# allenai/satlas-super-resolution

Hardware: AMD Instinct MI355X
Metric: G+D train-step images/sec (higher is better)
Workload: dtype fp32h

## Files before the change

### satlas_super_resolution_amd/csrc/conv_big_x3.hip

```cpp
#include "common.h"
#include <cstdlib>

namespace {

constexpr int XB_TH = 32, XB_TW = 16;
template <int KT> struct XbT {
    static constexpr int AROW = 80;
    static constexpr int VPP = 4;
    static constexpr int PH = XB_TH + KT - 1, PW = XB_TW + KT - 1, NPIX = PH * PW;
    static constexpr int PATCH = NPIX * AROW;
    static constexpr int WROWS = KT * KT * 64;
    static constexpr int WBYTES = WROWS * AROW;
    static constexpr int BUF = PATCH + WBYTES;
    static constexpr int BIAS = BUF;
    static constexpr int SLABS = BIAS + 256;
    static constexpr int LDS = SLABS + 4 * 32 * 272;
    static constexpr int NPV = (NPIX * VPP + 255) / 256;
    static constexpr int NWV = (WROWS * VPP + 255) / 256;
    static constexpr int NSTEP = KT * KT;
    static constexpr int TAIL = KT == 3 ? 2 : 1;
    static constexpr int LPS = (NPV + NWV + NSTEP - TAIL - 1) / (NSTEP - TAIL);
    static_assert(LDS <= 160 * 1024 && LPS <= 6, "LDS budget / load slots of a step");
};

#define XB_BAR() asm volatile("s_waitcnt lgkmcnt(0)\n\ts_barrier" ::: "memory")
#ifdef SSR_PROBE
#define XB_T() (__builtin_amdgcn_s_memtime())
#define XB_ACC(k, t0) do { const unsigned long long t1_ = XB_T(); xb_t[k] += t1_ - (t0); (t0) = t1_; } while (0)
#else
#define XB_T() 0ull
#define XB_ACC(k, t0) do { } while (0)
#endif
constexpr int XB_OOB = 0x7ffffff0;
constexpr int XB_SLAB_PITCH = 272, XB_SLAB = 32 * XB_SLAB_PITCH;
__device__ __forceinline__ __amdgpu_buffer_rsrc_t xb_rsrc(const void* p, long bytes) {
    return __builtin_amdgcn_make_buffer_rsrc(const_cast<void*>(p), 0, (int)(bytes > 0x7fffff00L ? 0x7fffff00L : (bytes < 0 ? 0 : bytes)), 0x00020000);
}
template <int KT>
__device__ __forceinline__ void xb_pixel(int w, int m, int s, int& row, int& col) {
    row = 8 * w + 2 * m + (s >> 4);
    col = s < 16 ? s : ((s + 32 - (XB_TW + KT - 1)) & 15);
}
__device__ __forceinline__ void xb_split4(const u32x4& v, uint2& hi, uint2& lo) {
    const f32x4 f = __builtin_bit_cast(f32x4, v);
    bf16x4 h, l;
#pragma unroll
    for (int k = 0; k < 4; ++k) {
        h[k] = (__bf16)f[k];
        l[k] = (__bf16)(f[k] - (float)h[k]);
    }
    hi = __builtin_bit_cast(uint2, h);
    lo = __builtin_bit_cast(uint2, l);
}

template <int KT, bool H = false>
__device__ __forceinline__ void conv_bigx3_body(const ssr_conv_desc& d) {
    using T = XbT<KT>;
    constexpr int AROW = T::AROW, VPP = T::VPP, PW = T::PW, NPIX = T::NPIX, PATCH = T::PATCH, NPV = T::NPV, NWV = T::NWV, NSTEP = T::NSTEP;
    extern __shared__ __attribute__((aligned(16))) char smem[];
    const int tid = threadIdx.x, lane = tid & 63, wave = tid >> 6;
    const int i = lane & 31, g = lane >> 5;
    const int tiles_x = (d.Gw + XB_TW - 1) / XB_TW, tiles_y = (d.Gh + XB_TH - 1) / XB_TH;
    const int tpi = tiles_x * tiles_y, G = gridDim.x / tpi;
    const int tp = blockIdx.x % tpi, n0 = blockIdx.x / tpi;
    const int tx_i = tp % tiles_x, ty_i = tp / tiles_x;
    const int nimg = (d.N - n0 + G - 1) / G;
    const int gy0 = ty_i * XB_TH, gx0 = tx_i * XB_TW;
    const int co0 = blockIdx.y * 64;
    const int upshift = d.up == 2 ? 1 : 0;
    const int LH = d.Hi << upshift, LW = d.Wi << upshift;
    const int nchunks = (d.Cin + 15) / 16;
    const int wchunk = KT * KT * d.CoutPad * 64;
    const int T_ = nimg * nchunks;
    const int ximg = d.Hi * d.Wi * d.x.cs * 4, oimg = d.Ho * d.Wo;

    unsigned long long xb_t[8] = {0, 0, 0, 0, 0, 0, 0, 0}, xb_t0 = XB_T();
    const unsigned long long xb_start = xb_t0;
    (void)xb_t; (void)xb_start;
    float* bias_lds = reinterpret_cast<float*>(smem + T::BIAS);
    if (tid < 64) bias_lds[tid] = (d.bias && co0 + tid < d.Cout) ? d.bias[co0 + tid] * (H ? SSR_F32H_WSCALE : 1.f) : 0.f;

    const bool s2d = KT == 2 && d.s2d != 0;
    const int cpc_shift = s2d ? 31 - __builtin_clz((unsigned)(d.Cin >> 6)) : 0;
    const int x_cs = d.x.cs, x_Wi = d.Wi, x_Cin = d.Cin;
    static_assert((T::WROWS * VPP) % 256 == 0, "no partial weight vector");
    const int p4 = tid >> 2, part4 = tid & 3;
    const int plo0 = p4 * AROW + part4 * 8;
    const int wlo0 = PATCH + p4 * AROW + part4 * 16;
    const int wgo0 = (co0 + p4) * 64 + part4 * 16, wstep = d.CoutPad * 64;
    constexpr int PTAIL = NPIX * VPP - (NPV - 1) * 256;
    int pgo[NPV];
    unsigned pmk[KT == 2 ? NPV : 1];
    const int climit = s2d ? 0x7fffffff : x_Cin - (tid % VPP) * 4;
#pragma unroll
    for (int q = 0; q < NPV; ++q) {
        const int v = tid + q * 256;
        const int pix = v / VPP, part = v % VPP;
        const int py = pix / PW, px = pix - py * PW;
        const int ly = gy0 + py - d.pad_y, lx = gx0 + px - d.pad_x;
        if constexpr (KT == 2) {
            if (s2d) {
                const int sy = 2 * ly - 1, sx = 2 * lx - 1;
                const bool y0 = sy >= 0 && sy < d.Hi, y1 = sy + 1 >= 0 && sy + 1 < d.Hi;
                const bool x0 = sx >= 0 && sx < d.Wi, x1 = sx + 1 >= 0 && sx + 1 < d.Wi;
                pmk[q] = v < NPIX * VPP ? (unsigned)(y0 && x0) | (unsigned)(y0 && x1) << 1 | (unsigned)(y1 && x0) << 2 | (unsigned)(y1 && x1) << 3 : 0u;
                pgo[q] = ((sy * d.Wi + sx) * d.x.cs + d.x.coff + part * 4) * 4 + (d.Wi + 1) * d.x.cs * 4;
            } else {
                const bool ok = v < NPIX * VPP && ly >= 0 && ly < LH && lx >= 0 && lx < LW;
                pmk[q] = ok ? 1u : 0u;
                pgo[q] = ok ? (((ly >> upshift) * d.Wi + (lx >> upshift)) * d.x.cs + d.x.coff + part * 4) * 4 : XB_OOB;
            }
        } else {
            const bool ok = v < NPIX * VPP && ly >= 0 && ly < LH && lx >= 0 && lx < LW;
            pgo[q] = ok ? (((ly >> upshift) * d.Wi + (lx >> upshift)) * d.x.cs + d.x.coff + part * 4) * 4 : XB_OOB;
        }
    }
    const long xbias = s2d ? (long)(d.Wi + 1) * d.x.cs * 4 : 0;
    const __amdgpu_buffer_rsrc_t rsx = xb_rsrc(reinterpret_cast<const char*>(d.x.p) - xbias, (long)d.N * ximg + xbias),
                                 rsw = xb_rsrc(d.w, (long)nchunks * wchunk);
    u32x4 rp[NPV], rw[NWV];
    struct LoadPos { int q, c0, xs, ws; };
    auto load_pos = [&](int nn, int c) {
        LoadPos p;
        p.c0 = c * 16;
        if constexpr (KT == 2) {
            p.q = s2d ? c >> cpc_shift : 0;
            p.xs = nn * ximg + (s2d ? (((p.q >> 1) * x_Wi + (p.q & 1)) * x_cs + ((c - (p.q << cpc_shift)) << 4)) * 4 : p.c0 * 4);
        } else {
            p.q = 0;
            p.xs = nn * ximg + p.c0 * 4;
        }
        p.ws = c * wchunk;
        return p;
    };
    auto load_one = [&](const LoadPos& lp, auto jc) {
        constexpr int j = decltype(jc)::value;
        if constexpr (j < NPV) {
            bool ok = lp.c0 < climit;
            if constexpr (KT == 2) ok = ok && ((pmk[j] >> lp.q) & 1u);
            rp[j] = __builtin_amdgcn_raw_buffer_load_b128(rsx, ok ? pgo[j] : XB_OOB, lp.xs, 0);
        } else {
            rw[j - NPV] = __builtin_amdgcn_raw_buffer_load_b128(rsw, wgo0, lp.ws + (j - NPV) * wstep, 0);
        }
    };
    auto load_chunk = [&](int nn, int c) { const LoadPos lp = load_pos(nn, c); static_for<0, NPV + NWV>([&](auto jc) { load_one(lp, jc); }); };
    auto store_chunk = [&]() {
        static_for<0, NPV>([&](auto jc) {
            constexpr int j = decltype(jc)::value;
            uint2 hi, lo;
            split_f32x4<H>(rp[j], hi, lo);
            if (j + 1 < NPV || tid < PTAIL) {
                *reinterpret_cast<uint2*>(smem + plo0 + j * 64 * AROW) = hi;
                *reinterpret_cast<uint2*>(smem + plo0 + j * 64 * AROW + 32) = lo;
            }
        });
        static_for<0, NWV>([&](auto jc) {
            constexpr int j = decltype(jc)::value;
            *reinterpret_cast<u32x4*>(smem + wlo0 + j * 64 * AROW) = rw[j];
        });
    };

    int a_off[4];
#pragma unroll
    for (int m = 0; m < 4; ++m) {
        int row, col;
        xb_pixel<KT>(wave, m, i, row, col);
        a_off[m] = (row * PW + col) * AROW + g * 16;
    }
    const int b_off = PATCH + i * AROW + g * 16;
    const int co_l = 4 * g;

    load_chunk(n0, 0);
    __syncthreads();
    XB_ACC(1, xb_t0);
    f32x16 acc[4][2];
    auto acc_init = [&]() {
#pragma unroll
        for (int t = 0; t < 2; ++t)
#pragma unroll
            for (int q4 = 0; q4 < 4; ++q4) {
                const f32x4 bq = *reinterpret_cast<const f32x4*>(bias_lds + t * 32 + 8 * q4 + co_l);
#pragma unroll
                for (int e = 0; e < 4; ++e)
#pragma unroll
                    for (int m = 0; m < 4; ++m) acc[m][t][4 * q4 + e] = bq[e];
            }
    };

    char* slab = smem + T::SLABS + wave * XB_SLAB;
    auto epilogue_impl = [&](int nn, auto opsc, auto y01c) __attribute__((always_inline)) {
        constexpr bool OPS = decltype(opsc)::value, Y01 = decltype(y01c)::value;
        const long obytes = (long)d.N * oimg * 4;
        const __amdgpu_buffer_rsrc_t rs_r1 = xb_rsrc(d.r1.p, d.r1.p ? obytes * d.r1.cs : 0), rs_r2 = xb_rsrc(d.r2.p, d.r2.p ? obytes * d.r2.cs : 0),
                                     rs_m = xb_rsrc(d.m.p, d.m.p ? obytes * d.m.cs : 0), rs_y = xb_rsrc(d.y.p, obytes * d.y.cs),
                                     rs_y0 = xb_rsrc(d.y0.p, d.y0.p ? obytes * d.y0.cs : 0), rs_y1 = xb_rsrc(d.y1.p, d.y1.p ? obytes * d.y1.cs : 0);
        const bool has_r1 = d.r1.p != nullptr, has_r2 = d.r2.p != nullptr, has_m = d.m.p != nullptr, has_acc = d.accumulate != 0,
                   has_y0 = d.y0.p != nullptr, has_y1 = d.y1.p != nullptr, m_relu = d.m_relu != 0;
        const float slope = d.act == SSR_ACT_LRELU ? 0.2f : d.act == SSR_ACT_RELU ? 0.f : 1.f;
        const float alpha = d.alpha, beta1 = has_r1 ? d.beta1 : 0.f, beta2 = has_r2 ? d.beta2 : 0.f, gacc = has_acc ? 1.f : 0.f;
        const int y_cs = d.y.cs, y_co = d.y.coff, y0_cs = d.y0.cs, y0_co = d.y0.coff, y1_cs = d.y1.cs, y1_co = d.y1.coff;
        const int r1_cs = d.r1.cs, r1_co = d.r1.coff, r2_cs = d.r2.cs, r2_co = d.r2.coff, m_cs = d.m.cs, m_co = d.m.coff;
        const int Gh = d.Gh, Gw = d.Gw, oys = d.oys, oyo = d.oyo, oxs = d.oxs, oxo = d.oxo, Wo = d.Wo;
        const int pimg = nn * oimg;
        const int hp = lane >> 4, c = co0 + (lane & 15) * 4;
        const bool cok = c < d.Cout;
#pragma unroll
        for (int m = 0; m < 4; ++m) {
            int po[8];
#pragma unroll
            for (int h = 0; h < 8; ++h) {
                int row, col;
                xb_pixel<KT>(wave, m, 4 * h + hp, row, col);
                const int gy = gy0 + row, gx = gx0 + col;
                const bool ok = gy < Gh && gx < Gw;
                const int cy = gy < Gh ? gy : Gh - 1, cx = gx < Gw ? gx : Gw - 1;
                po[h] = (pimg + (cy * oys + oyo) * Wo + cx * oxs + oxo) | (ok && cok ? 0 : (int)0x80000000);
            }
#pragma unroll
            for (int t = 0; t < 2; ++t)
#pragma unroll
                for (int q4 = 0; q4 < 4; ++q4) {
                    const f32x4 v = {acc[m][t][4 * q4], acc[m][t][4 * q4 + 1], acc[m][t][4 * q4 + 2], acc[m][t][4 * q4 + 3]};
                    *reinterpret_cast<f32x4*>(slab + i * XB_SLAB_PITCH + (t * 32 + 8 * q4 + co_l) * 4) = v;
                }
#pragma unroll
            for (int hh = 0; hh < 2; ++hh) {
                u32x4 q1[OPS ? 4 : 1], q2[OPS ? 4 : 1], qa[OPS ? 4 : 1], qm[OPS ? 4 : 1];
                if constexpr (OPS) {
#pragma unroll
                    for (int h4 = 0; h4 < 4; ++h4) {
                        const int pp = po[4 * hh + h4] & 0x7fffffff;
                        q1[h4] = __builtin_amdgcn_raw_buffer_load_b128(rs_r1, cok && has_r1 ? (pp * r1_cs + r1_co + c) * 4 : XB_OOB, 0, 0);
                        q2[h4] = __builtin_amdgcn_raw_buffer_load_b128(rs_r2, cok && has_r2 ? (pp * r2_cs + r2_co + c) * 4 : XB_OOB, 0, 0);
                        qa[h4] = __builtin_amdgcn_raw_buffer_load_b128(rs_y, cok && has_acc ? (pp * y_cs + y_co + c) * 4 : XB_OOB, 0, 0);
                        qm[h4] = __builtin_amdgcn_raw_buffer_load_b128(rs_m, cok && has_m ? (pp * m_cs + m_co + c) * 4 : XB_OOB, 0, 0);
                    }
                }
#pragma unroll
                for (int h4 = 0; h4 < 4; ++h4) {
                    const int h = 4 * hh + h4;
                    f32x4 a = *reinterpret_cast<const f32x4*>(slab + (4 * h + hp) * XB_SLAB_PITCH + (lane & 15) * 16);
                    if constexpr (H) a *= SSR_F32H_UNSCALE;
                    const bool ok = po[h] >= 0;
                    const int pp = po[h] & 0x7fffffff;
                    f32x4 v, s0, s1;
#pragma unroll
                    for (int e = 0; e < 4; ++e) {
                        float x = fmaxf(a[e], slope * a[e]) * alpha;
                        s0[e] = x;
                        if constexpr (OPS) {
                            x += beta1 * __builtin_bit_cast(f32x4, q1[h4])[e] + beta2 * __builtin_bit_cast(f32x4, q2[h4])[e] + gacc * __builtin_bit_cast(f32x4, qa[h4])[e];
                            s1[e] = x;
                            const float mv = __builtin_bit_cast(f32x4, qm[h4])[e];
                            const float f = m_relu ? (mv > 0.f ? 1.f : 0.f) : lrelu_grad_from_out(mv);
                            x *= has_m ? f : 1.f;
                        } else {
                            s1[e] = x;
                        }
                        v[e] = x;
                    }
                    if constexpr (Y01) {
                        __builtin_amdgcn_raw_buffer_store_b128(__builtin_bit_cast(u32x4, s0), rs_y0, ok && has_y0 ? (pp * y0_cs + y0_co + c) * 4 : XB_OOB, 0, 0);
                        __builtin_amdgcn_raw_buffer_store_b128(__builtin_bit_cast(u32x4, s1), rs_y1, ok && has_y1 ? (pp * y1_cs + y1_co + c) * 4 : XB_OOB, 0, 0);
                    }
                    __builtin_amdgcn_raw_buffer_store_b128(__builtin_bit_cast(u32x4, v), rs_y, ok ? (pp * y_cs + y_co + c) * 4 : XB_OOB, 0, 0);
                }
            }
        }
    };
    auto epilogue = [&](int nn) __attribute__((always_inline)) {
        const bool ops = d.r1.p != nullptr || d.r2.p != nullptr || d.m.p != nullptr || d.accumulate != 0;
        const bool y01 = d.y0.p != nullptr || d.y1.p != nullptr;
        if (ops) {
            if (y01) epilogue_impl(nn, std::true_type{}, std::true_type{});
            else epilogue_impl(nn, std::true_type{}, std::false_type{});
        } else {
            if (y01) epilogue_impl(nn, std::false_type{}, std::true_type{});
            else epilogue_impl(nn, std::false_type{}, std::false_type{});
        }
    };

    auto chunk = [&](int c, bool stored, int nn1, int c1, auto hnc) __attribute__((always_inline)) {
        constexpr bool has_next = decltype(hnc)::value;
        xb_t0 = XB_T();
        if (!stored) {
            if (c > 0) XB_BAR();
            XB_ACC(2, xb_t0);
            store_chunk();
            XB_ACC(3, xb_t0);
        }
        XB_BAR();
        XB_ACC(4, xb_t0);
        const LoadPos lp1 = load_pos(nn1, c1);
        bf16x8 wq[2][2][2], pq[2][4][2];
        auto issue1 = [&](auto sc, auto kc) {
            constexpr int s_ = decltype(sc)::value, k = decltype(kc)::value;
            if constexpr (k < 4)
                wq[s_ & 1][k >> 1][k & 1] = *reinterpret_cast<const bf16x8*>(smem + b_off + (s_ * 64 + (k >> 1) * 32) * AROW + (k & 1) * 32);
            else
                pq[s_ & 1][(k - 4) >> 1][k & 1] =
                    *reinterpret_cast<const bf16x8*>(smem + a_off[(k - 4) >> 1] + ((s_ / KT) * PW + s_ % KT) * AROW + (k & 1) * 32);
        };
        static_for<0, 12>([&](auto kc) { issue1(std::integral_constant<int, 0>{}, kc); });
        static_for<0, NSTEP>([&](auto sc) {
            constexpr int s_ = decltype(sc)::value;
            static_for<0, 24>([&](auto kc) {
                constexpr int k = decltype(kc)::value, m = k / 6, t = (k % 6) / 3, p = k % 3;
                acc[m][t] = split_mfma<H>(wq[s_ & 1][t][p == 0 ? 1 : 0], pq[s_ & 1][m][p == 1 ? 1 : 0], acc[m][t]);
                __builtin_amdgcn_sched_barrier(0);
                if constexpr (k < 12) {
                    if constexpr (s_ + 1 < NSTEP) issue1(std::integral_constant<int, s_ + 1>{}, kc);
                } else if constexpr (has_next && (k & 1) == 0 && (k - 12) / 2 < T::LPS) {
                    constexpr int j = s_ * T::LPS + (k - 12) / 2;
                    if constexpr (j < NPV + NWV) load_one(lp1, std::integral_constant<int, j>{});
                }
                __builtin_amdgcn_sched_barrier(0);
            });
        });
        __builtin_amdgcn_sched_barrier(0);
        XB_ACC(5, xb_t0);
        xb_t[7] += 1;
    };
    int gc = 0;
    for (int k = 0; k < nimg; ++k) {
        const int nn = n0 + k * G;
        const bool last_img = k + 1 == nimg;
        acc_init();
        for (int c = 0; c < (last_img ? nchunks - 1 : nchunks); ++c, ++gc) {
            const bool last_c = c + 1 == nchunks;
            chunk(gc, k > 0 && c == 0, last_c ? nn + G : nn, last_c ? 0 : c + 1, std::true_type{});
        }
        if (!last_img) {
            xb_t0 = XB_T();
            XB_BAR();
            XB_ACC(2, xb_t0);
            store_chunk();
            XB_ACC(3, xb_t0);
            epilogue(nn);
            XB_ACC(6, xb_t0);
        }
    }
    const int nl = n0 + (nimg - 1) * G;
    chunk(gc, nimg > 1 && nchunks == 1, nl, 0, std::false_type{});
    xb_t0 = XB_T();
    epilogue(nl);
    XB_ACC(6, xb_t0);
#ifdef SSR_PROBE
    if (tid == 0) {
        xb_t[0] = XB_T() - xb_start;
        const int b = (blockIdx.z * gridDim.y + blockIdx.y) * gridDim.x + blockIdx.x;
        for (int k = 0; k < 8; ++k) g_probe[b * 8 + k] = xb_t[k];
    }
#endif
    (void)T_;
}

struct ssr_conv_desc4x { ssr_conv_desc d[4]; };
template <int KT>
__global__ __launch_bounds__(256, 1) void conv_bigx3_kernel4(const ssr_conv_desc4x p) {
    conv_bigx3_body<KT>(p.d[blockIdx.z]);
}
template <int KT>
__global__ __launch_bounds__(256, 1) void conv_bigh3_kernel4(const ssr_conv_desc4x p) {
    conv_bigx3_body<KT, true>(p.d[blockIdx.z]);
}

template <int KT, bool H = false>
int launch_bigx3(const ssr_conv_desc* ds, int n, hipStream_t st) {
    constexpr int lds = XbT<KT>::LDS;
    const ssr_conv_desc& d = ds[0];
    const int tpi = ((d.Gh + XB_TH - 1) / XB_TH) * ((d.Gw + XB_TW - 1) / XB_TW);
    static const int ncu = [] { int dev = 0, v = 256; if (hipGetDevice(&dev) == hipSuccess && hipDeviceGetAttribute(&v, hipDeviceAttributeMultiprocessorCount, dev) != hipSuccess) v = 256; return v > 0 ? v : 256; }();
    int G = d.N;
    {
        const long per_img = (long)tpi * (d.CoutPad / 64) * n;
        long best = -1;
        for (int g = 1; g <= d.N; ++g) {
            const long rounds = (per_img * g + ncu - 1) / ncu, cost = rounds * ((d.N + g - 1) / g);
            const long key = (cost << 24) | (rounds << 12) | (4095 - (g > 4095 ? 4095 : g));
            if (best < 0 || key < best) { best = key; G = g; }
        }
    }
    if (const char* e = getenv("SSR_CONV_BIG_G")) {
        const int g = atoi(e);
        if (g >= 1) G = g < d.N ? g : d.N;
    }
    const int tiles = tpi * G;
    auto kern = H ? conv_bigh3_kernel4<KT> : conv_bigx3_kernel4<KT>;
    static bool attr_done[SSR_MAX_DEVICES] = {};
    const int attr_dev = ssr_device_ordinal();
    if (!attr_done[attr_dev]) {
        hipError_t e = hipFuncSetAttribute(reinterpret_cast<const void*>(kern), hipFuncAttributeMaxDynamicSharedMemorySize, lds);
        if (e != hipSuccess) return (int)e;
        attr_done[attr_dev] = true;
    }
    ssr_conv_desc4x p;
    for (int k = 0; k < 4; ++k) p.d[k] = ds[k < n ? k : 0];
    hipLaunchKernelGGL(kern, dim3(tiles, d.CoutPad / 64, n), dim3(256), lds, st, p);
    SSR_LAUNCH_CHECK();
    return SSR_OK;
}

}

bool ssr_conv_bigx3_shape_ok(const ssr_conv_desc& d) {
    if ((d.dtype != SSR_F32X3 && d.dtype != SSR_F32H) || d.fix_list) return false;
    const bool k3 = d.KH == 3 && d.KW == 3 && d.pad_y == 1 && d.pad_x == 1;
    const bool k2 = d.KH == 2 && d.KW == 2 && (d.pad_y == 0 || d.pad_y == 1) && (d.pad_x == 0 || d.pad_x == 1);
    if (!(k3 || k2) || d.stride != 1 || d.x2.p) return false;
    if (d.Cin < 8 || (d.CoutPad % 64) != 0 || (d.Cout % 4) != 0) return false;
    if (d.s2d) {
        const int cpc = d.Cin / 64;
        if (!k2 || d.pad_y != 0 || d.pad_x != 0 || d.up != 1 || (d.Cin % 64) != 0 || cpc < 1 || (cpc & (cpc - 1)) != 0) return false;
        if ((d.Hi % 2) != 0 || (d.Wi % 2) != 0 || d.Gh != d.Hi / 2 || d.Gw != d.Wi / 2) return false;
    } else if (d.Gh != (d.Hi << (d.up == 2)) || d.Gw != (d.Wi << (d.up == 2))) return false;
    if (d.r1.p && d.r1_nc < d.Cout) return false;
    if (d.r2.p && d.r2_nc < d.Cout) return false;
    if (d.m.p && !(d.m_c0 == 0 && d.m_c1 >= d.Cout)) return false;
    const long lim = 0x7fffff00L;
    const long xin = ((long)d.N * d.Hi * d.Wi + d.Wi + 1) * d.x.cs * 4, npo = (long)d.N * d.Ho * d.Wo * 4;
    if (xin > lim || npo * d.y.cs > lim || (d.y0.p && npo * d.y0.cs > lim) || (d.y1.p && npo * d.y1.cs > lim) || (d.r1.p && npo * d.r1.cs > lim) ||
        (d.r2.p && npo * d.r2.cs > lim) || (d.m.p && npo * d.m.cs > lim))
        return false;
    if ((long)((d.Cin + 15) / 16) * d.KH * d.KW * d.CoutPad * 64 > lim) return false;
    auto al16 = [](const ssr_view& v) { return !v.p || ((v.cs % 4) == 0 && (v.coff % 4) == 0 && ((uintptr_t)v.p % 16) == 0); };
    return d.x.p && d.y.p && al16(d.x) && al16(d.y) && al16(d.y0) && al16(d.y1) && al16(d.r1) && al16(d.r2) && al16(d.m);
}

bool ssr_conv_bigx3_qualifies(const ssr_conv_desc& d) {
    static const bool off = [] { const char* e = getenv("SSR_X3_BIGTILE"); return e && e[0] == '0'; }();
    if (off || !ssr_conv_bigx3_shape_ok(d) || d.KH != 3) return false;
    const long per_img = (long)((d.Gh + XB_TH - 1) / XB_TH) * ((d.Gw + XB_TW - 1) / XB_TW) * (d.CoutPad / 64);
    return per_img >= 4 && d.Gh >= 24;
}

bool ssr_conv_bigx3_try(const ssr_conv_desc& d, hipStream_t st, int* rc, bool force) {
    if (force ? !ssr_conv_bigx3_shape_ok(d) : !ssr_conv_bigx3_qualifies(d)) return false;
    if (d.dtype == SSR_F32H) *rc = d.KH == 3 ? launch_bigx3<3, true>(&d, 1, st) : launch_bigx3<2, true>(&d, 1, st);
    else *rc = d.KH == 3 ? launch_bigx3<3>(&d, 1, st) : launch_bigx3<2>(&d, 1, st);
    return true;
}

bool ssr_conv_bigx3_batch_try(const ssr_conv_desc* ds, int n, hipStream_t st, int* rc) {
    const char* e = getenv("SSR_X3_BIGTILE2");
    const bool off = e && e[0] == '0', always = e && e[0] == '2';
    if (off || n < 1 || n > 4) return false;
    for (int k = 0; k < n; ++k)
        if (!ssr_conv_bigx3_shape_ok(ds[k]) || ds[k].dtype != SSR_F32X3 || ds[k].KH != 2 || ds[k].s2d) return false;
    const ssr_conv_desc& d = ds[0];
    for (int k = 1; k < n; ++k)
        if (ds[k].N != d.N || ds[k].Gh != d.Gh || ds[k].Gw != d.Gw || ds[k].CoutPad != d.CoutPad || ds[k].Cin != d.Cin || ds[k].Hi != d.Hi || ds[k].Wi != d.Wi ||
            ds[k].up != d.up)
            return false;
    const long per_img = (long)((d.Gh + XB_TH - 1) / XB_TH) * ((d.Gw + XB_TW - 1) / XB_TW) * (d.CoutPad / 64) * n;
    if (!always && (per_img < 8 || d.Gh < 24)) return false;
    *rc = launch_bigx3<2>(ds, n, st);
    return true;
}
```

Measured before the change: 1186.

## Double-buffer input patches in big conv kernel to overlap loads with MFMA

Adds a pipelined variant of the big conv kernel in which the input patch, and for 2x2 kernels also the weights, live in two LDS buffers. The next chunk's global loads, hi/lo split and LDS stores are interleaved with the current chunk's MFMAs, which removes the per-chunk serialisation of load, barrier and compute. The epilogue slab reuses the idle patch buffer, and the leaky-ReLU product is precomputed in one epilogue case. This is on by default through an env toggle. In exchange it raises LDS use and register pressure and adds complex scheduling.

```diff
diff --git a/satlas_super_resolution_amd/csrc/conv_big_x3.hip b/satlas_super_resolution_amd/csrc/conv_big_x3.hip
--- a/satlas_super_resolution_amd/csrc/conv_big_x3.hip
+++ b/satlas_super_resolution_amd/csrc/conv_big_x3.hip
@@ -21,6 +21,13 @@
     static constexpr int TAIL = KT == 3 ? 2 : 1;
     static constexpr int LPS = (NPV + NWV + NSTEP - TAIL - 1) / (NSTEP - TAIL);
     static_assert(LDS <= 160 * 1024 && LPS <= 6, "LDS budget / load slots of a step");
+    static constexpr bool WDB = KT == 2;
+    static constexpr int PWB = 2 * PATCH;
+    static constexpr int PBIAS = PWB + (WDB ? 2 : 1) * WBYTES;
+    static constexpr int PLDS = PBIAS + 256;
+    static constexpr int PSTEPS = (NPV + 2) / 3;
+    static_assert(PLDS <= 160 * 1024 && 4 * 32 * 272 <= PATCH && (PATCH % 16) == 0, "pipelined LDS budget / slabs in a patch buffer");
+    static_assert(PSTEPS < NSTEP && 2 * NWV <= 24, "pipelined store slots");
 };
 
 #define XB_BAR() asm volatile("s_waitcnt lgkmcnt(0)\n\ts_barrier" ::: "memory")
@@ -41,6 +48,27 @@
     row = 8 * w + 2 * m + (s >> 4);
     col = s < 16 ? s : ((s + 32 - (XB_TW + KT - 1)) & 15);
 }
+template <bool H> __device__ __forceinline__ void xb_split2(float a, float b, uint32_t& hi, uint32_t& lo) {
+    if constexpr (H) {
+        typedef _Float16 f16x2 __attribute__((ext_vector_type(2)));
+        f16x2 h, l;
+        h[0] = (_Float16)a;
+        h[1] = (_Float16)b;
+        l[0] = (_Float16)(a - (float)h[0]);
+        l[1] = (_Float16)(b - (float)h[1]);
+        hi = __builtin_bit_cast(uint32_t, h);
+        lo = __builtin_bit_cast(uint32_t, l);
+    } else {
+        typedef __bf16 bf16x2 __attribute__((ext_vector_type(2)));
+        bf16x2 h, l;
+        h[0] = (__bf16)a;
+        h[1] = (__bf16)b;
+        l[0] = (__bf16)(a - (float)h[0]);
+        l[1] = (__bf16)(b - (float)h[1]);
+        hi = __builtin_bit_cast(uint32_t, h);
+        lo = __builtin_bit_cast(uint32_t, l);
+    }
+}
 __device__ __forceinline__ void xb_split4(const u32x4& v, uint2& hi, uint2& lo) {
     const f32x4 f = __builtin_bit_cast(f32x4, v);
     bf16x4 h, l;
@@ -53,7 +81,7 @@
     lo = __builtin_bit_cast(uint2, l);
 }
 
-template <int KT, bool H = false>
+template <int KT, bool H = false, bool PIPE = false>
 __device__ __forceinline__ void conv_bigx3_body(const ssr_conv_desc& d) {
     using T = XbT<KT>;
     constexpr int AROW = T::AROW, VPP = T::VPP, PW = T::PW, NPIX = T::NPIX, PATCH = T::PATCH, NPV = T::NPV, NWV = T::NWV, NSTEP = T::NSTEP;
@@ -77,7 +105,7 @@
     unsigned long long xb_t[8] = {0, 0, 0, 0, 0, 0, 0, 0}, xb_t0 = XB_T();
     const unsigned long long xb_start = xb_t0;
     (void)xb_t; (void)xb_start;
-    float* bias_lds = reinterpret_cast<float*>(smem + T::BIAS);
+    float* bias_lds = reinterpret_cast<float*>(smem + (PIPE ? T::PBIAS : T::BIAS));
     if (tid < 64) bias_lds[tid] = (d.bias && co0 + tid < d.Cout) ? d.bias[co0 + tid] * (H ? SSR_F32H_WSCALE : 1.f) : 0.f;
 
     const bool s2d = KT == 2 && d.s2d != 0;
@@ -170,9 +198,11 @@
     const int b_off = PATCH + i * AROW + g * 16;
     const int co_l = 4 * g;
 
-    load_chunk(n0, 0);
-    __syncthreads();
-    XB_ACC(1, xb_t0);
+    if constexpr (!PIPE) {
+        load_chunk(n0, 0);
+        __syncthreads();
+        XB_ACC(1, xb_t0);
+    }
     f32x16 acc[4][2];
     auto acc_init = [&]() {
 #pragma unroll
@@ -243,10 +273,15 @@
                     if constexpr (H) a *= SSR_F32H_UNSCALE;
                     const bool ok = po[h] >= 0;
                     const int pp = po[h] & 0x7fffffff;
-                    f32x4 v, s0, s1;
+                    f32x4 v, s0, s1, s0p;
+                    if constexpr (OPS && Y01) {
+#pragma unroll
+                        for (int e = 0; e < 4; ++e) s0p[e] = fmaxf(a[e], slope * a[e]) * alpha;
+                        asm("" : "+v"(s0p));
+                    }
 #pragma unroll
                     for (int e = 0; e < 4; ++e) {
-                        float x = fmaxf(a[e], slope * a[e]) * alpha;
+                        float x = OPS && Y01 ? s0p[e] : fmaxf(a[e], slope * a[e]) * alpha;
                         s0[e] = x;
                         if constexpr (OPS) {
                             x += beta1 * __builtin_bit_cast(f32x4, q1[h4])[e] + beta2 * __builtin_bit_cast(f32x4, q2[h4])[e] + gacc * __builtin_bit_cast(f32x4, qa[h4])[e];
@@ -321,6 +356,121 @@
         XB_ACC(5, xb_t0);
         xb_t[7] += 1;
     };
+    const int wlo_p = p4 * AROW + part4 * 16, b_off_p = i * AROW + g * 16;
+    auto chunk_p = [&](int c, const LoadPos& lp2, auto hnc) __attribute__((always_inline)) {
+        constexpr bool has_next = decltype(hnc)::value;
+        xb_t0 = XB_T();
+        if (c > 0) XB_BAR();
+        XB_ACC(2, xb_t0);
+        const int pb = (c & 1) * PATCH, pbn = PATCH - pb;
+        const int wb = T::PWB + (T::WDB ? (c & 1) * T::WBYTES : 0), wbn = T::PWB + (T::WDB ? T::WBYTES - (c & 1) * T::WBYTES : 0);
+        const int pw = wb + b_off_p;
+        int pa[4];
+#pragma unroll
+        for (int m = 0; m < 4; ++m) pa[m] = pb + a_off[m];
+        bf16x8 wq[2][2][2], pq[2][4][2];
+        uint32_t sh[2], sl[2];
+        auto issue1 = [&](auto sc, auto kc) {
+            constexpr int s_ = decltype(sc)::value, k = decltype(kc)::value;
+            if constexpr (k < 4)
+                wq[s_ & 1][k >> 1][k & 1] = *reinterpret_cast<const bf16x8*>(smem + pw + (s_ * 64 + (k >> 1) * 32) * AROW + (k & 1) * 32);
+            else
+                pq[s_ & 1][(k - 4) >> 1][k & 1] =
+                    *reinterpret_cast<const bf16x8*>(smem + pa[(k - 4) >> 1] + ((s_ / KT) * PW + s_ % KT) * AROW + (k & 1) * 32);
+        };
+        static_for<0, 12>([&](auto kc) { issue1(std::integral_constant<int, 0>{}, kc); });
+        static_for<0, NSTEP>([&](auto sc) {
+            constexpr int s_ = decltype(sc)::value;
+            static_for<0, 24>([&](auto kc) {
+                constexpr int k = decltype(kc)::value, m = k / 6, t = (k % 6) / 3, p = k % 3;
+                acc[m][t] = split_mfma<H>(wq[s_ & 1][t][p == 0 ? 1 : 0], pq[s_ & 1][m][p == 1 ? 1 : 0], acc[m][t]);
+                __builtin_amdgcn_sched_barrier(0);
+                if constexpr (s_ + 1 < NSTEP && k < 12) {
+                    issue1(std::integral_constant<int, s_ + 1>{}, kc);
+                } else if constexpr (has_next && s_ + 1 < NSTEP) {
+                    constexpr int j = 3 * s_ + (k - 12) / 4, ph = (k - 12) % 4;
+                    if constexpr (j < NPV && (k - 12) / 4 < 3) {
+                        if constexpr (ph < 2) {
+                            const f32x4 f = __builtin_bit_cast(f32x4, rp[j]);
+                            xb_split2<H>(f[2 * ph], f[2 * ph + 1], sh[ph], sl[ph]);
+                        } else if constexpr (ph == 2) {
+                            if (j + 1 < NPV || tid < PTAIL) {
+                                *reinterpret_cast<uint2*>(smem + pbn + plo0 + j * 64 * AROW) = uint2{sh[0], sh[1]};
+                                *reinterpret_cast<uint2*>(smem + pbn + plo0 + j * 64 * AROW + 32) = uint2{sl[0], sl[1]};
+                            }
+                        } else {
+                            load_one(lp2, std::integral_constant<int, j>{});
+                        }
+                    }
+                } else if constexpr (has_next) {
+                    constexpr int j = k / 2;
+                    if constexpr (j < NWV) {
+                        if constexpr ((k & 1) == 0) *reinterpret_cast<u32x4*>(smem + wbn + wlo_p + j * 64 * AROW) = rw[j];
+                        else load_one(lp2, std::integral_constant<int, NPV + j>{});
+                    }
+                }
+                __builtin_amdgcn_sched_barrier(0);
+            });
+            if constexpr (has_next && !T::WDB && s_ + 2 == NSTEP) {
+                XB_ACC(5, xb_t0);
+                XB_BAR();
+                XB_ACC(3, xb_t0);
+                __builtin_amdgcn_sched_barrier(0);
+            }
+        });
+        __builtin_amdgcn_sched_barrier(0);
+        XB_ACC(5, xb_t0);
+        xb_t[7] += 1;
+    };
+    if constexpr (PIPE) {
+        auto advance = [&](int& nn, int& c) { if (++c == nchunks) { c = 0; nn += G; if (nn >= d.N) nn = n0; } };
+        int ln = n0, lc = 0;
+        load_chunk(n0, 0);
+        static_for<0, NPV>([&](auto jc) {
+            constexpr int j = decltype(jc)::value;
+            uint2 hi, lo;
+            split_f32x4<H>(rp[j], hi, lo);
+            if (j + 1 < NPV || tid < PTAIL) {
+                *reinterpret_cast<uint2*>(smem + plo0 + j * 64 * AROW) = hi;
+                *reinterpret_cast<uint2*>(smem + plo0 + j * 64 * AROW + 32) = lo;
+            }
+        });
+        static_for<0, NWV>([&](auto jc) {
+            constexpr int j = decltype(jc)::value;
+            *reinterpret_cast<u32x4*>(smem + T::PWB + wlo_p + j * 64 * AROW) = rw[j];
+        });
+        advance(ln, lc);
+        load_chunk(ln, lc);
+        advance(ln, lc);
+        XB_BAR();
+        XB_ACC(1, xb_t0);
+        int gc = 0;
+        for (int k = 0; k < nimg; ++k) {
+            const int nn = n0 + k * G;
+            const bool last_img = k + 1 == nimg;
+            acc_init();
+            for (int c = 0; c < (last_img ? nchunks - 1 : nchunks); ++c, ++gc) {
+                chunk_p(gc, load_pos(ln, lc), std::true_type{});
+                advance(ln, lc);
+            }
+            if (!last_img) {
+                xb_t0 = XB_T();
+                XB_BAR();
+                XB_ACC(4, xb_t0);
+                slab = smem + ((gc - 1) & 1) * PATCH + wave * XB_SLAB;
+                epilogue(nn);
+                XB_ACC(6, xb_t0);
+            }
+        }
+        const int nl = n0 + (nimg - 1) * G;
+        chunk_p(gc, load_pos(ln, lc), std::false_type{});
+        xb_t0 = XB_T();
+        XB_BAR();
+        XB_ACC(4, xb_t0);
+        slab = smem + (gc & 1) * PATCH + wave * XB_SLAB;
+        epilogue(nl);
+        XB_ACC(6, xb_t0);
+    } else {
     int gc = 0;
     for (int k = 0; k < nimg; ++k) {
         const int nn = n0 + k * G;
@@ -345,6 +495,7 @@
     xb_t0 = XB_T();
     epilogue(nl);
     XB_ACC(6, xb_t0);
+    }
 #ifdef SSR_PROBE
     if (tid == 0) {
         xb_t[0] = XB_T() - xb_start;
@@ -358,16 +509,30 @@
 struct ssr_conv_desc4x { ssr_conv_desc d[4]; };
 template <int KT>
 __global__ __launch_bounds__(256, 1) void conv_bigx3_kernel4(const ssr_conv_desc4x p) {
-    conv_bigx3_body<KT>(p.d[blockIdx.z]);
+    conv_bigx3_body<KT, false, true>(p.d[blockIdx.z]);
 }
 template <int KT>
 __global__ __launch_bounds__(256, 1) void conv_bigh3_kernel4(const ssr_conv_desc4x p) {
+    conv_bigx3_body<KT, true, true>(p.d[blockIdx.z]);
+}
+template <int KT>
+__global__ __launch_bounds__(256, 1) void conv_bigx3_1b_kernel4(const ssr_conv_desc4x p) {
+    conv_bigx3_body<KT>(p.d[blockIdx.z]);
+}
+template <int KT>
+__global__ __launch_bounds__(256, 1) void conv_bigh3_1b_kernel4(const ssr_conv_desc4x p) {
     conv_bigx3_body<KT, true>(p.d[blockIdx.z]);
+}
+
+bool ssr_conv_bigx3_pipelined() {
+    static const bool on = [] { const char* e = getenv("SSR_XB_PIPE"); return !(e && e[0] == '0'); }();
+    return on;
 }
 
 template <int KT, bool H = false>
 int launch_bigx3(const ssr_conv_desc* ds, int n, hipStream_t st) {
-    constexpr int lds = XbT<KT>::LDS;
+    const bool pipe = ssr_conv_bigx3_pipelined();
+    const int lds = pipe ? XbT<KT>::PLDS : XbT<KT>::LDS;
     const ssr_conv_desc& d = ds[0];
     const int tpi = ((d.Gh + XB_TH - 1) / XB_TH) * ((d.Gw + XB_TW - 1) / XB_TW);
     static const int ncu = [] { int dev = 0, v = 256; if (hipGetDevice(&dev) == hipSuccess && hipDeviceGetAttribute(&v, hipDeviceAttributeMultiprocessorCount, dev) != hipSuccess) v = 256; return v > 0 ? v : 256; }();
@@ -386,7 +551,7 @@
         if (g >= 1) G = g < d.N ? g : d.N;
     }
     const int tiles = tpi * G;
-    auto kern = H ? conv_bigh3_kernel4<KT> : conv_bigx3_kernel4<KT>;
+    auto kern = pipe ? (H ? conv_bigh3_kernel4<KT> : conv_bigx3_kernel4<KT>) : (H ? conv_bigh3_1b_kernel4<KT> : conv_bigx3_1b_kernel4<KT>);
     static bool attr_done[SSR_MAX_DEVICES] = {};
     const int attr_dev = ssr_device_ordinal();
     if (!attr_done[attr_dev]) {
```

After: 1199 (median of 6 runs). 1.2% higher.
